# HIITMetagenomics/dsm-framework

Measured on AMD Instinct MI355X. Metric: enumerated substrings/sec (Emax=2.0), higher is better.
Workload: dtype u32

## Files before the change

### dsm-framework_amd/csrc/engine.hip

```cpp
#include <sched.h>

#include <algorithm>
#include <atomic>
#include <chrono>
#include <cmath>
#include <condition_variable>
#include <cstdlib>
#include <cstring>
#include <deque>
#include <map>
#include <functional>
#include <memory>
#include <mutex>
#include <sstream>
#include <thread>
#include <type_traits>

#include "common.h"
#include "scan.h"
#include "setorder.h"
#include "stream_parse.h"
#include "lfstep.h"
#include "entropy_tables.h"
#include "textemit.h"
// ... 194 lines not shown
#pragma unroll
        for (int g = 0; g < 8; ++g) {
            const u64 f = w[g] & (PACK_FMAX - 1);
            if (f) {
                const u32 lg = w[g] >> 13;
                l = l == 0xFF ? lg : (l == lg ? l : 5u);
                sumN += f;
                if (a.emax > 0) s += (double)(f + 1) * (double)__log2f((float)(f + 1));
            }
        }
    } else {
        for (u32 g = 0; g < a.d; ++g) {
            u64 f = (u64)x_freq<P>(x, g, v);
            if (f) {
                u32 lg = x_pl<P>(x, g, v) >> 4;
                l = l == 0xFF ? lg : (l == lg ? l : 5u);
                sumN += f;
                if (a.emax > 0) s += (double)(f + 1) * (double)__log2f((float)(f + 1));
            }
        }
    }
    if (l >= 1 && l <= 4) return false;
    if (a.emax > 0) {
        double e = (double)__log2f((float)sumN) - s / (double)sumN;
        if (e < a.emin - ENT_MARGIN || e > a.emax + ENT_MARGIN) return false;
    }
    return true;
}

constexpr u32 PW_CHUNK = 16;
constexpr u32 SREC_FIRST = 4u, SREC_LAST = 8u;
__device__ __forceinline__ uint2 child_path_word(const uint2 parent, u32 u, u32 plevel, u32 c) {
    const u32 r = plevel & (PW_CHUNK - 1);
    return r == 0 ? make_uint2(u, c) : make_uint2(parent.x, parent.y | (c << (2 * r)));
}

struct AdvanceOut {
    u32* slot;
    uint2* sa;
    uint2* pw;
    const uint2* parent_pw;
    const u32* width;
    u32 pw_after_slot;
    u32 plevel;
    u32 kshift;
    u32 cand_copy;
    u16* nT;
    u8* samechild;
    const u16* parent_nT;
    const u64* kplane;
    u64* kplane_w;
    u32* kcum;
    const u32* cnt4;
    u32* cnt_clear;
    u32 nbp;
    const u16* sinfo;
    u32 eval;
    u32 single;
    u32* const* rp;
    u32* rp0;
    const u64* const* splane;
    u32 rp_index;
    const u32* const* tpos;
    u32 nlocal, rank;
    u32 seg;
    u32 cap;
    u32* h_totals;
    u32 filter_on;
    FilterArgs fa;
    u64* candbits;
    u64* wsum;
    uint4* crec;
    u32 crec_cap;
};

struct PublishArgs {
    const u32* total;
    const u64* cand;
    const u8* cmax_base;
    u64 cmax_bpr;
    u32 cmax_world;
    u32* clear;
    u32* next;
    uint4* packet;
    u32 seq;
    uint4* bc_header;
    const u32* grand;
};
__global__ void publish_kernel(PublishArgs a) {
    __shared__ u32 wide;
    if (threadIdx.x == 0) wide = 0;
    __syncthreads();
    for (u32 r = threadIdx.x; r < a.cmax_world; r += blockDim.x) {
        const u64 m = *reinterpret_cast<const u64*>(a.cmax_base + (u64)r * a.cmax_bpr);
        if (m >= PACK_FMAX) atomicOr(&wide, m >= 65535 ? 3u : 2u);
    }
    const u32 tot = threadIdx.x == 0 ? *a.total : 0u;
    u64 cand = threadIdx.x == 0 && a.cand ? *a.cand : 0ull;
    if (threadIdx.x == 0 && a.grand) { const u64 c = (u64)(*a.grand - tot); cand = c | (c << 32); }
    __syncthreads();
    if (a.clear && threadIdx.x < 4) a.clear[threadIdx.x] = 0;
    if (threadIdx.x == 0) {
        if (a.next) { a.next[0] = tot; a.next[1] = wide; }
        const uint4 pk = make_uint4(a.seq, tot | ((wide & 1u) << 31) | ((wide >> 1) << 30), (u32)cand, (u32)(cand >> 32));
        if (a.bc_header) *a.bc_header = make_uint4(BC_OK, pk.y, 0u, 0u);
        *a.packet = pk;
// ... 203 lines not shown
    if (!o.single) o.samechild[u] = (u8)same;
#pragma unroll
    for (int c = 0; c < 4; ++c) {
        if (((pres >> c) & 1u) && vj[c] < o.cap) {
            if (o.slot) o.slot[vj[c]] = 4u * u + (u32)c;
            if (pw) pw[vj[c]] = child_path_word(mypw, u, o.plevel, (u32)c);
            if (o.sa) o.sa[vj[c]] = make_uint2(u, (u32)c | ((pres & ((1u << c) - 1u)) ? 0u : SREC_FIRST) | ((pres >> (c + 1)) ? 0u : SREC_LAST));
            if (!o.single) o.nT[vj[c]] = (u16)nT4[c];
        }
    }
    if (o.single) {
#pragma unroll
        for (int c = 0; c < 4; ++c)
            if (((pres >> c) & 1u) && vj[c] < o.cap) o.rp0[vj[c]] = (u32)c * o.seg + w * 64u + (u32)__popcll(up[c] & lt);
        return;
    }
    for (u32 sl = 0; sl < o.nlocal && pres && (o.tpos || o.rp_index); ++sl) {
        u32* rp = o.rp[sl];
        if (o.tpos) {
            const u32 m = x_pl<P>(x, o.rank * o.nlocal + sl, u) & 15u;
            const u32 h = m ? o.tpos[sl][u] : 0u;
#pragma unroll
            for (int c = 0; c < 4; ++c)
                if (((pres >> c) & 1u) && vj[c] < o.cap) rp[vj[c]] = ((m >> c) & 1u) ? h + (u32)__popc(m & ((1u << c) - 1u)) : DEAD;
        } else {
            const u64* sp = o.splane[sl] + (size_t)w * 4;
#pragma unroll
            for (int c = 0; c < 4; ++c) {
                if (!((pres >> c) & 1u) || vj[c] >= o.cap) continue;
                const u64 mine = sp[c];
                rp[vj[c]] = ((mine >> lane) & 1) ? (u32)c * o.seg + w * 64u + (u32)__popcll(mine & lt) : DEAD;
            }
        }
    }
}

template <typename P>
__global__ __launch_bounds__(256) void advance_single_kernel(Xchg x, AdvanceOut o) {
    const int lane = threadIdx.x & 63;
    const u32 F = (u32)x.F;
    const u32 nw = (F + 63) >> 6;
    const u32 tile = (u32)__builtin_amdgcn_readfirstlane((int)(xcd_block() * 4 + (threadIdx.x >> 6)));
    if (tile >= o.nbp) return;
    const u64 lt = (1ull << lane) - 1;
    const u64* __restrict__ line = o.kplane + (size_t)tile * 32;
    uint2 mypw[4];
#pragma unroll
    for (int q = 0; q < 4; ++q) {
        const u32 u = (tile * 4 + (u32)q) * 64 + lane;
        mypw[q] = o.parent_pw[u < F ? u : 0u];
    }
    u64 copyw = 0;
    if (lane < 32) copyw = line[lane];
    u32 cum[4];
#pragma unroll
    for (int c = 0; c < 4; ++c) cum[c] = o.cnt4[(size_t)c * o.nbp + tile];
    u64 up[4][4];
#pragma unroll
    for (int q = 0; q < 4; ++q)
#pragma unroll
        for (int c = 0; c < 4; ++c) up[q][c] = tile * 4 + (u32)q < nw ? line[q * 8 + c] : 0ull;
    {
        const u32 q = (u32)lane >> 3, j = (u32)lane & 7u, w = tile * 4 + q;
        if (lane < 32 && w < nw) {
            if (j < 4) o.kplane_w[(size_t)w * 4 + j] = copyw;
            else if (o.cand_copy && j == 4) o.candbits[w] = copyw;
            else if (o.cand_copy && j == 5) o.wsum[w] = copyw;
        }
    }
    const u32 r = o.plevel & (PW_CHUNK - 1);
    u32 kc = 0;
    u32 cbase = 0;
    u64 cbq[4] = {0, 0, 0, 0};
    u32 ncq[4] = {0, 0, 0, 0};
    u64 fq[4] = {0, 0, 0, 0};
    if (o.crec) {
        cbase = o.cnt4[(size_t)4 * o.nbp + tile] - o.cnt4[(size_t)4 * o.nbp];
#pragma unroll
        for (int q = 0; q < 4; ++q) {
            if (tile * 4 + (u32)q < nw) { cbq[q] = line[q * 8 + 4]; ncq[q] = (u32)line[q * 8 + 5]; }
            const u32 u = (tile * 4 + (u32)q) * 64 + lane;
            if ((cbq[q] >> lane) & 1ull) fq[q] = (u64)x_freq<P>(x, 0, u);
        }
    }
#pragma unroll
    for (int q = 0; q < 4; ++q) {
        const u32 w = tile * 4 + (u32)q, u = w * 64 + lane;
        const uint2 ppw = mypw[q];
        if (o.crec && cbq[q]) {
            const u32 k = cbase + bits_below_lane(cbq[q]);
            if (((cbq[q] >> lane) & 1ull) && k < o.crec_cap) o.crec[k] = make_uint4(u, 0u, (u32)fq[q], (u32)(fq[q] >> 32));
        }
        cbase += ncq[q];
#pragma unroll
        for (int c = 0; c < 4; ++c) {
            const u64 m = up[q][c];
            if (lane == q * 4 + c) kc = cum[c];
            const u32 below = bits_below_lane(m);
            const u32 vj = cum[c] + below;
            if (((m >> lane) & 1ull) && vj < o.cap) {
                o.rp0[vj] = (u32)c * o.seg + w * 64u + below;
                o.pw[vj] = r == 0 ? make_uint2(u, (u32)c) : make_uint2(ppw.x, ppw.y | ((u32)c << (2 * r)));
            }
            cum[c] += (u32)__popcll(m);
        }
    }
    if (lane < 16 && tile * 4 + ((u32)lane >> 2) < nw) o.kcum[(size_t)tile * 16 + lane] = kc;
}

__global__ __launch_bounds__(256) void lite_count_kernel(const u64* __restrict__ kplane, u32 nw, u32* __restrict__ cnt4, u32 nbp, u32 kshift, u32 cand_row = 0) {
    const u32 tile = blockIdx.x * 64 + (threadIdx.x >> 2), c = threadIdx.x & 3;
    if (tile >= nbp) return;
    u32 s = 0, nc = 0;
    if (cand_row && tile * 4 + c < nw) nc = (u32)kplane[((size_t)(tile * 4 + c) << 3) + 5];
#pragma unroll
    for (u32 q = 0; q < 4; ++q) {
        const u32 w = tile * 4 + q;
        if (w < nw) s += (u32)__popcll(kplane[((size_t)w << kshift) + c]);
    }
    cnt4[(size_t)c * nbp + tile] = s;
    if (cand_row) {
        nc += __shfl_xor(nc, 1, 64);
        nc += __shfl_xor(nc, 2, 64);
        if (c == 0) cnt4[(size_t)4 * nbp + tile] = nc;
    }
}
__global__ __launch_bounds__(256) void lite_slot_kernel(const u64* __restrict__ kplane, u32 F, const u32* __restrict__ cnt4, u32 nbp, u32 single_tile,
                                                        u32* __restrict__ slot, u32 cap) {
    const int lane = threadIdx.x & 63;
    const u32 nw = (F + 63) >> 6;
    const u32 tile = xcd_block();
    const u32 wi = threadIdx.x >> 6, w = tile * 4 + wi;
    if (w >= nw) return;
    const u32 u = w * 64 + lane;
    u32 base = 0;
#pragma unroll
    for (int c = 0; c < 4; ++c) {
        u32 before = 0, all = 0;
#pragma unroll
        for (u32 q = 0; q < 4; ++q) {
            const u32 wq = tile * 4 + q;
            const u32 t = wq < nw ? (u32)__popcll(kplane[(size_t)wq * 4 + c]) : 0u;
            before += q < wi ? t : 0u;
            all += t;
        }
        const u64 up = kplane[(size_t)w * 4 + c];
        const u32 first = (single_tile ? base : cnt4[(size_t)c * nbp + tile]) + before;
        base += all;
        const u32 vj = first + (u32)__popcll(up & ((1ull << lane) - 1));
        if (u < F && ((up >> lane) & 1) && vj < cap) slot[vj] = 4u * u + (u32)c;
    }
}

template <typename P>
__global__ __launch_bounds__(256) void order_kernel(u32 F, Xchg x, const u16* __restrict__ nT, const u64* __restrict__ order, Kids kids,
                                                    u64* __restrict__ order_next) {
    __shared__ u32 qn;
    __shared__ u32 qu[256];
    __shared__ u64 qm[256], qo[256];
    if (threadIdx.x == 0) qn = 0;
    __syncthreads();
    const u32 u = blockIdx.x * blockDim.x + threadIdx.x;
    if (u < F) {
        const u32 cnt = nT[u];
        const u64 ord = order[u];
        u64 mbyid = 0;
        u32 um = 0;
        if (x_is_nm8(x)) {
            u32 w[8];
            x_words8(x, u, w);
#pragma unroll
            for (int g = 0; g < 8; ++g) { const u32 m = (w[g] >> 9) & 15u; mbyid |= (u64)m << (4 * g); um |= m; }
        } else {
            for (u32 k = 0; k < cnt; ++k) {
                const u32 r = (u32)((ord >> (4 * k)) & 15);
                const u32 m = x_pl<P>(x, r, u) & 15u;
                mbyid |= (u64)m << (4 * r);
                um |= m;
// ... 1185 lines not shown
    tpos[i] = fc[r] + __popc(full & 15u & (low - 1));
}

#define EARENA_GET(var, T, n)                                                                       \
    do {                                                                                            \
        (var) = ea->template get<T>(n);                                                             \
        if (!(var)) return fail(DSM_E_CAPACITY, "device arena exhausted: use a longer prefix or a larger arena_bytes"); \
    } while (0)

template <typename P>
class Engine {
  public:
    std::vector<const dsm_index*> idx;
    std::vector<const dsm_trie*> tries;
    bool trie_mode = false;
    dsm_params prm;
    bool stream_mode = false;
    int nlocal = 0, world = 1, rank = 0;
    u32 d = 1;
    hipStream_t st = 0;
    int device = 0;

    u32 Fcap = 0;
    bool multi = false;
    bool owner_mode = false;
    bool is_owner = true;
    int owner = 0;
    u8* bc_buf = nullptr;
    u32* lite_slot[2] = {nullptr, nullptr};
    uint2* sa[2] = {nullptr, nullptr};
    u32 pub_seq = 0;
    u32 Seg = 0;
    u32 Rcap = 0;
    u32 FcapW = 0, SegW = 0, RcapW = 0;
    u32 seg_of(bool compact) const { return compact ? Seg : SegW; }
    u32* d_pub_tot = nullptr; u64* d_pub_cmax = nullptr;
    std::vector<P*> rec[2];
    std::vector<u32*> rp[2];
    std::vector<u32*> tpos;
    std::vector<u64*> splane;
    u32** d_rp_tab[2] = {nullptr, nullptr};
    u32** d_tpos_tab = nullptr;
    u64** d_splane_tab = nullptr;
    bool spec_mode = false;
    u32* d_dyn = nullptr;
    bool node_major(bool w9) const { return w9 && nlocal > 1 && nlocal <= 8 && !trie_mode; }
    u32 dense_min = 1u << 18;
    bool self_mode = false;
    std::vector<u64*> splane2;
    u8* xsend = nullptr;
    u8* xrecv[2] = {nullptr, nullptr};
    u64 bpr_cap = 0;
    u32 *cnt4 = nullptr, *scan_tmp = nullptr;
    u32* cntraw = nullptr;
    LfGeometry lfgeo{256, 16};
    u16* sinfo = nullptr;
    u16* nT[2] = {nullptr, nullptr};
    u8* samechild = nullptr;
    u64* order[2] = {nullptr, nullptr};
    u16* order16[2] = {nullptr, nullptr};
    u64 *cand_wsum = nullptr, *cand_wscan = nullptr, *scan_tmp64 = nullptr;
    u64* d_counters = nullptr;
    u32* d_totals = nullptr;
    u64* d_totals64 = nullptr;
    u32* h_totals = nullptr;
    u32* h_bounds = nullptr;
    u64* h_childmax = nullptr;
    std::vector<void*> owned;
    size_t owned_bytes = 0;
    Arena arena;
    Arena carena;
    Arena earena;
    Arena* ea = nullptr;
    hipEvent_t ev0 = nullptr, ev1 = nullptr;
    std::vector<hipEvent_t> evpool;
    dsm_stats stats;
    u32 splits = 0;
    Emitter emitter;
    dsm_text_sink text_sink_ = nullptr;

    ~Engine() {
        for (void* p : owned) (void)hipFree(p);
        if (h_totals) (void)hipHostFree(h_totals);
        if (h_bounds) (void)hipHostFree(h_bounds);
        if (h_childmax) (void)hipHostFree(h_childmax);
        if (ev0) (void)hipEventDestroy(ev0);
        if (ev1) (void)hipEventDestroy(ev1);
        {
            std::lock_guard<std::mutex> lk(g_expand_chain.mu);
            for (auto& kv : g_expand_chain.dev)
                if (kv.second.owner == this) kv.second = ExpandChain::Link();
        }
        for (hipEvent_t e : evpool) (void)hipEventDestroy(e);
        if (copy_stream) (void)hipStreamDestroy(copy_stream);
        if (fill_done) (void)hipEventDestroy(fill_done);
        for (auto e : chunk_filled) if (e) (void)hipEventDestroy(e);
        if (bounds_landed) (void)hipEventDestroy(bounds_landed);
    }

    template <class T> int dalloc(T*& p, size_t n) {
        void* q = nullptr;
        hipError_t e = hipMalloc(&q, (n ? n : 1) * sizeof(T));
        if (e != hipSuccess) return fail(DSM_E_NOMEM, std::string("hipMalloc: ") + hipGetErrorString(e));
        owned.push_back(q);
        owned_bytes += ((n ? n : 1) * sizeof(T) + 4095) & ~(size_t)4095;
        p = (T*)q;
        return 0;
    }

    int init(dsm_index* const* ix, int n, const dsm_params& p, bool stream) {
        device = ix[0]->device;
        u64 nsum = 0, nmax = 0;
        for (int k = 0; k < n; ++k) {
            if (ix[k]->device != device) return fail(DSM_E_INVAL, "all local indexes must live on one device");
            idx.push_back(ix[k]);
            nsum += ix[k]->meta.n;
            nmax = ix[k]->meta.n > nmax ? ix[k]->meta.n : nmax;
        }
        return init_common(n, p, stream, nsum, nmax);
    }
    int init_tries(dsm_trie* const* tr, int n, const dsm_params& p) {
        device = tr[0]->device;
        trie_mode = true;
        u64 nsum = 0, nmax = 0;
        for (int k = 0; k < n; ++k) {
            if (tr[k]->device != device) return fail(DSM_E_INVAL, "all tries must live on one device");
            tries.push_back(tr[k]);
            nsum += tr[k]->nodes + 16;
            nmax = tr[k]->nodes + 16 > nmax ? tr[k]->nodes + 16 : nmax;
        }
        return init_common(n, p, false, nsum, nmax);
    }
    int init_common(int n, const dsm_params& p, bool stream, u64 nsum, u64 nmax) {
        memset(&stats, 0, sizeof stats);
        prm = p;
        stream_mode = stream;
        nlocal = n;
        world = p.world_size > 1 ? (int)p.world_size : 1;
        rank = world > 1 ? (int)p.rank : 0;
        multi = world > 1 || (p.allgather && getenv("DSM_FORCE_EXCHANGE"));
        if (world > 1 && !p.allgather) return fail(DSM_E_INVAL, "world_size > 1 needs an allgather callback");
        owner_mode = multi && p.owner_mode != 0;
        if (owner_mode) {
            if (!p.gather || !p.bcast) return fail(DSM_E_INVAL, "owner_mode needs the gather and bcast callbacks");
            if ((int)p.owner_rank >= world) return fail(DSM_E_INVAL, "owner_rank >= world_size");
            if (stream || trie_mode) return fail(DSM_E_INVAL, "owner_mode is for mining indexes");
            owner = (int)p.owner_rank;
            is_owner = rank == owner;
        }
        if (rank >= world) return fail(DSM_E_INVAL, "rank >= world_size");
        if (n > MAX_LOCAL) return fail(DSM_E_INVAL, "at most 273 local samples per process");
        d = (u32)(world * nlocal);
        if (d > 273) return fail(DSM_E_INVAL, "too many samples (MAX_READERS 273, metaserver.cpp:19)");
        st = (hipStream_t)p.stream;
        DSM_HIP(hipSetDevice(device));
        size_t free_b = 0, total_b = 0;
        DSM_HIP(hipMemGetInfo(&free_b, &total_b));
        if (const char* e = getenv("DSM_DENSE_MIN")) dense_min = (u32)atol(e);
        spec_mode = d == 1 && !trie_mode && !multi;
        if (spec_mode) { if (int rc = dalloc(d_dyn, (size_t)4)) return rc; }
        self_mode = d > 1 && !trie_mode;
        if (owner_mode && !self_mode) return fail(DSM_E_INVAL, "owner_mode needs handles derived in the LF-step kernel (several samples)");
        const u64 fbound = (world > 1 ? (u64)d * nmax : nsum) + 16;
        u64 budget = p.arena_bytes ? p.arena_bytes : (u64)(free_b * 0.7);
        if (!p.arena_bytes) {
            u64 want = (256ull << 20) + 32ull * nsum * (u64)world;
            if (want < budget) budget = want;
        }
        if (budget > free_b) budget = (u64)(free_b * 0.9);
        const bool small_rec = sizeof(P) == 8 && !trie_mode;
        const u64 rec_b = small_rec ? 32 : REC_FIELDS * sizeof(P) + 1;
        u64 perF = (u64)nlocal * (2 * rec_b * 4 + 2 * 4 + 4 + 1)
                   + (u64)nlocal * (sizeof(P) + 1)
                   + 2ull * d * (sizeof(P) + 1)
                   + 2 * (2 + 1 + 8) + 1 + 16 + 64 + (d > 13 ? 4ull * d : 0) + (d > 1 ? 8 : 0);
        u64 fc = budget * (nlocal > 1 && !p.arena_bytes ? 2 : 1) / 3 / perF;
        if (fc > (1u << 28) - TILE) fc = (1u << 28) - TILE;
        if (fc < 512) return fail(DSM_E_NOMEM, "not enough device memory for the frontier buffers");
        if (fc > fbound) fc = fbound < 1024 ? 1024 : fbound;
        Fcap = (u32)fc;
        bpr_cap = (((u64)nlocal * Fcap * (sizeof(P) + 1) + 15) & ~15ull) + 16;
        if (p.exchange_send && p.exchange_recv && multi) {
            if (p.exchange_bytes < 1024) return fail(DSM_E_INVAL, "exchange buffers too small");
            u64 cap_slots = (p.exchange_bytes - 32) / ((u64)nlocal * (sizeof(P) + 1));
            if (cap_slots < Fcap) Fcap = (u32)cap_slots;
            bpr_cap = p.exchange_bytes;
            xsend = (u8*)p.exchange_send;
            xrecv[0] = (u8*)p.exchange_recv;
            xrecv[1] = (u8*)p.exchange_recv + (size_t)world * bpr_cap;
        } else {
            if (int rc = dalloc(xrecv[0], (size_t)world * bpr_cap)) return rc;
            if (int rc = dalloc(xrecv[1], (size_t)world * bpr_cap)) return rc;
            if (multi) { if (int rc = dalloc(xsend, (size_t)bpr_cap)) return rc; }
        }
        if (multi) {
            u64 mine = Fcap, agreed = 0;
            if (int rc = agree_min(mine, &agreed)) return rc;
            Fcap = (u32)agreed;
        }
        if (int rc = alloc_levels(small_rec)) return rc;
        const size_t used = owned_bytes;
        u64 arena_b = budget > used ? budget - used : 0;
        const u64 floor_b = p.arena_bytes ? (1u << 20) : (64u << 20);
        if (arena_b < floor_b) arena_b = floor_b;
        if (multi) {
            u64 agreed = 0;
            if (int rc = agree_min(arena_b, &agreed)) return rc;
            arena_b = agreed;
        }
        if (int rc = dalloc(arena.base, arena_b)) return rc;
        arena.cap = arena_b;
// ... 17 lines not shown
        DSM_HIP(hipEventCreateWithFlags(&ev1, hipEventDisableSystemFence));
        return 0;
    }

    int alloc_levels(bool small_rec) {
        Seg = (Fcap + TILE - 1) / TILE * TILE;
        Rcap = 4 * Seg;
        SegW = Seg; FcapW = Fcap;
        if (small_rec) {
            SegW = (u32)((u64)Seg * 32 / (REC_FIELDS * sizeof(P) + 1)) / TILE * TILE;
            if (SegW < TILE) SegW = TILE;
            FcapW = SegW < Fcap ? SegW : Fcap;
        }
        RcapW = 4 * SegW;
        const size_t rec_n = std::max(rec_elems<P>(RcapW), small_rec ? (size_t)Rcap * 32 / sizeof(P) : (size_t)0);
        const size_t ntile = Seg / TILE, nwave = ntile * 4;
        const u64 slots = (u64)Fcap * 4;
        for (int s = 0; s < nlocal; ++s) {
            P *a = nullptr, *b = nullptr;
            u32 *r0, *r1, *tp = nullptr;
            u64* pln = nullptr;
            if (!trie_mode) {
                if (int rc = dalloc(a, rec_n)) return rc;
                if (int rc = dalloc(b, rec_n)) return rc;
                if (int rc = dalloc(pln, nwave * (d == 1 ? 8 : 4))) return rc;
            } else {
                if (int rc = dalloc(tp, (size_t)Fcap)) return rc;
            }
            if (int rc = dalloc(r0, (size_t)Fcap)) return rc;
            if (int rc = dalloc(r1, (size_t)Fcap)) return rc;
            u64* pln2 = nullptr;
            if (self_mode) { if (int rc = dalloc(pln2, nwave * 4)) return rc; }
            splane2.push_back(pln2);
            rec[0].push_back(a); rec[1].push_back(b); rp[0].push_back(r0); rp[1].push_back(r1); tpos.push_back(tp); splane.push_back(pln);
        }
        for (int k = 0; k < 2; ++k) {
            if (int rc = dalloc(d_rp_tab[k], (size_t)nlocal)) return rc;
            DSM_HIP(hipMemcpy(d_rp_tab[k], rp[k].data(), (size_t)nlocal * sizeof(u32*), hipMemcpyHostToDevice));
        }
        if (int rc = dalloc(d_tpos_tab, (size_t)nlocal)) return rc;
        DSM_HIP(hipMemcpy(d_tpos_tab, tpos.data(), (size_t)nlocal * sizeof(u32*), hipMemcpyHostToDevice));
        if (int rc = dalloc(d_splane_tab, (size_t)nlocal)) return rc;
        DSM_HIP(hipMemcpy(d_splane_tab, splane.data(), (size_t)nlocal * sizeof(u64*), hipMemcpyHostToDevice));
        if (int rc = dalloc(cnt4, 5 * ntile + 8)) return rc;
        if (stream_mode)
            for (int k = 0; k < 2; ++k) if (int rc = dalloc(sa[k], (size_t)Fcap + 64)) return rc;
        if (owner_mode) {
            if (int rc = dalloc(bc_buf, 16 + 32 * nwave + 64)) return rc;
            for (int k = 0; k < 2; ++k) if (int rc = dalloc(lite_slot[k], (size_t)Fcap + 64)) return rc;
        }
        if (d == 1 && !trie_mode) {
            if (int rc = dalloc(cntraw, 5 * ntile + 8)) return rc;
            DSM_HIP(hipMemset(cntraw, 0, (5 * ntile + 8) * sizeof(u32)));
        }
        if (int rc = lf_step_geometry(sizeof(P) == 8, device, &lfgeo)) return rc;
        if (d > 1 || trie_mode) { if (int rc = dalloc(sinfo, (size_t)slots)) return rc; }
        if (int rc = dalloc(scan_tmp, scan_tmp_elems(5 * ntile) + 8)) return rc;
        for (int k = 0; k < 2; ++k) {
            if (int rc = dalloc(nT[k], Fcap)) return rc;
            if (int rc = dalloc(order[k], Fcap)) return rc;
        }
        if (d > 13)
            for (int k = 0; k < 2; ++k)
                if (int rc = dalloc(order16[k], (size_t)Fcap * d)) return rc;
        if (int rc = dalloc(samechild, Fcap)) return rc;
        if (int rc = dalloc(cand_wsum, nwave + 8)) return rc;
        if (int rc = dalloc(cand_wscan, nwave + 8)) return rc;
        if (int rc = dalloc(scan_tmp64, scan_tmp_elems(nwave) + 8)) return rc;
        if (int rc = dalloc(d_counters, (size_t)COUNTER_SHARDS * 8 + KEEP_FREQS / 64)) return rc;
        {
            std::vector<u32> kt(KEEP_FREQS / 32, ~0u);
            if (d == 1 && !trie_mode && prm.emax > 0) {
                const double* terms = term_table();
                const double* logn = logn_table();
                for (u32 f = 0; f < KEEP_FREQS; ++f) {
                    const u64 sumN = 1ull + f;
                    const double sl = f < TERM_TAB ? terms[f] : (double)((u64)f + 1) * log((double)((u64)f + 1)) / LN2;
                    const double e = (sumN < LOGN_TAB ? logn[sumN] : log((double)sumN) / LN2) - sl / (double)sumN;
                    if (e < prm.emin || e > prm.emax) kt[f >> 5] &= ~(1u << (f & 31));
                }
            }
            DSM_HIP(hipMemcpy(d_counters + (size_t)COUNTER_SHARDS * 8, kt.data(), kt.size() * sizeof(u32), hipMemcpyHostToDevice));
        }
        if (int rc = dalloc(d_totals, 8)) return rc;
        if (int rc = dalloc(d_totals64, 4)) return rc;
        if (int rc = dalloc(d_pub_tot, 8)) return rc;
        if (int rc = dalloc(d_pub_cmax, (size_t)(world > 0 ? world : 1))) return rc;
        DSM_HIP(hipHostMalloc((void**)&h_totals, 320 * sizeof(u32)));
        DSM_HIP(hipHostMalloc((void**)&h_bounds, 2 * (EmitSet::MAX_CHUNKS + 1) * sizeof(u32)));
        DSM_HIP(hipHostMalloc((void**)&h_childmax, (size_t)(world > 0 ? world : 1) * sizeof(u64)));
        return 0;
    }

    int agree_min(u64 mine, u64* out) {
        u8* send = xsend;
        DSM_HIP(hipMemcpyAsync(send, &mine, sizeof(u64), hipMemcpyHostToDevice, st));
        if (prm.allgather(prm.allgather_ctx, send, xrecv[0], sizeof(u64), (void*)st)) return fail(DSM_E_SINK, "allgather callback failed");
        std::vector<u64> all((size_t)world);
        DSM_HIP(hipMemcpyAsync(all.data(), xrecv[0], (size_t)world * sizeof(u64), hipMemcpyDeviceToHost, st));
        DSM_HIP(hipStreamSynchronize(st));
        u64 m = all[0];
        for (u64 v : all) m = v < m ? v : m;
        *out = m;
        return 0;
    }

// ... 41 lines not shown
            if (hipMemcpyAsync(e->bc_buf, hdr, 16, hipMemcpyHostToDevice, e->st) == hipSuccess) (void)hipStreamSynchronize(e->st);
            (void)e->prm.bcast(e->prm.owner_ctx, e->owner, e->bc_buf, bytes, (void*)e->st);
        }
    };

    u32 col_bytes(bool w16, bool w9) const { return w9 ? 2u : (w16 ? 3u : (u32)sizeof(P) + 1); }
    u64 level_bytes(u32 F, bool w16, bool w9) const { return (((u64)nlocal * F * col_bytes(w16, w9) + 15) & ~15ull) + 16; }
    static size_t bcast_bytes(u32 F) { return 16 + (size_t)((F + 63) >> 6) * 32; }
    u32 level_cap(bool w16) const { return w16 ? Fcap : FcapW; }
    int check_width(u32 Fn, bool w16) {
        if (Fn > level_cap(w16)) return fail(DSM_E_CAPACITY, "frontier wider than the device buffers: use a longer prefix or a larger arena_bytes");
        return 0;
    }
    u32 decode_level(u32 word, bool* w16, bool* w9) const {
        *w16 = !(word >> 31) && !trie_mode;
        *w9 = *w16 && !((word >> 30) & 1u);
        return word & 0x3FFFFFFFu;
    }
    int upload_order(int k, const u16* ro, size_t n) {
        if (d <= 13) {
            u64 ord = 0;
            for (size_t i = 0; i < n; ++i) ord |= (u64)ro[i] << (4 * i);
            DSM_HIP(hipMemcpyAsync(order[k], &ord, sizeof(u64), hipMemcpyHostToDevice, st));
        } else {
            DSM_HIP(hipMemcpyAsync(order16[k], ro, n * sizeof(u16), hipMemcpyHostToDevice, st));
        }
        return 0;
    }

    struct Walk {
        std::string prefix;
        RunOpts o;
        std::vector<LevelHost> L;
        u32 order_mode = 0;
        bool emitting = false;
        bool emit_failed = false;
        bool trace = false;
        size_t nev = 0;
        u32 F = 1, depth = 0;
        bool w16 = false, w9 = false;
        BcastGuard owed;
        explicit Walk(Engine* e) : owed(e) {}
        int cur() const { return (int)(depth & 1); }
    };
    struct Sweep {
        Xchg x;
        size_t mark = 0;
        u32* slot = nullptr;
        bool filtered = false;
        u32 crec_cap = 0;
        u32 Fn = 0;
        bool w16 = false, w9 = false;
        bool spec_hit = false;
    };

    int run(const char* prefix_c, dsm_tuple_sink tsink, dsm_byte_sink bsink, void* ctx, const RunOpts& o = RunOpts()) {
        Walk w(this);
        w.prefix = prefix_c ? prefix_c : "";
        w.o = o;
        for (char ch : w.prefix)
            if (ch != 'A' && ch != 'C' && ch != 'G' && ch != 'T')
                return fail(DSM_E_INVAL, "prefix must be over A,C,G,T");
        DSM_HIP(hipSetDevice(device));
        for (int s_ = 0; s_ < nlocal && !trie_mode; ++s_)
            if (!idx[s_]->dev.blk) return fail(DSM_E_INVAL, "an index of this miner is offloaded: dsm_index_reload first");
        arena.off = 0;
        earena.off = 0;
        carena.off = 0;
        w.emitting = o.emit;
        w.L.reserve(512);
        DSM_HIP(hipMemsetAsync(d_counters, 0, (size_t)COUNTER_SHARDS * 8 * sizeof(u64), st));
        if (cntraw) DSM_HIP(hipMemsetAsync(cntraw, 0, (4 * (size_t)(Seg / TILE) + 8) * sizeof(u32), st));
        DSM_HIP(hipEventRecord(ev0, st));
        if (int rc = root_level(w)) return rc;
        w.order_mode = (d < 2 || prm.pmax == 1) ? 0u : (d <= 13 ? 1u : 2u);
        stats.pair_order_exact = 1;
        w.trace = getenv("DSM_TRACE_LEVELS") != nullptr;
        DSM_HIP(hipMemsetAsync(multi ? xsend : xrecv[0], 0, XHDR, st));
        if (int rc = launch_lf(w, 0, 1, w.w16, w.w9, w.L[0].slot)) return rc;
        while (true) {
            if (int rc = exchange(w)) return rc;
            if (owner_mode && !is_owner) {
                bool more = false;
                if (int rc = client_level(w, &more)) return rc;
                if (!more) break;
                continue;
            }
            if (owner_mode) { if (int rc = owner_precheck(w)) return rc; }
            Sweep s;
            LevelHost child;
            if (int rc = advance(w, s)) return rc;
            if (int rc = publish(w, s)) return rc;
            if (int rc = commit(w, s, child)) return rc;
            if (int rc = capture_level(w, s.Fn, child.slot, child.pw)) return rc;
            if (s.filtered) {
                int erc = emit_store(w.L[w.depth], w.F, w.depth, s.x, w.cur(), w.order_mode, s.crec_cap);
                if (erc == DSM_E_CAPACITY && multi) { w.emit_failed = true; w.emitting = false; }
                else if (erc) return erc;
            }
            DSM_HIP(hipGetLastError());
            if (pend.submit && (w.F >= 200000u || w.depth >= 24)) { if (int rc = flush_pending()) return rc; }
            count_level(w);
            if (!s.Fn) break;
            w.L.push_back(child);
            step(w, s.Fn, s.w16, s.w9);
            if (w.L.size() > 60000) return fail(DSM_E_CAPACITY, "trie deeper than 60000 levels");
        }
        timeline("levels done", w.prefix.c_str());
        if (int rc = flush_pending()) return rc;
        if (int rc = finish_prefix(w, tsink, bsink, ctx)) return rc;
        if (w.o.last && pend.submit) {
            DSM_HIP(hipEventSynchronize(bounds_landed));
            if (int rc = flush_pending()) return rc;
        }
        return read_back(w);
    }

    int root_level(Walk& w) {
        const char* bases = "ACGT";
        for (int s = 0; s < nlocal && trie_mode; ++s) {
            const u32 zero = 0;
            DSM_HIP(hipMemcpyAsync(rp[0][s], &zero, sizeof(u32), hipMemcpyHostToDevice, st));
            stats.reported += tries[s]->nodes;
        }
        for (int s = 0; s < nlocal && !trie_mode; ++s) {
// ... 231 lines not shown
            ARENA_GET(me.clen, u8, F);
            hipLaunchKernelGGL((keep_kernel<P>), grid_for(F), dim3(256), 0, st, F, x, sa[cur], me.srec, me.clen);
        }
        if (!stream_mode && w.emitting && depth >= 1 && depth >= w.o.emit_lo && depth <= w.o.emit_hi) {
            int erc = emit_alloc(me, F);
            if (erc == DSM_E_CAPACITY && multi) { w.emit_failed = true; w.emitting = false; }
            else if (erc) return erc;
            else s.filtered = true;
        }
        s.mark = arena.off;
        const bool keep_slot = self_mode, keep_pw = !stream_mode;
        const size_t wcap = (size_t)F * 4 < Fcap ? (size_t)F * 4 : Fcap;
        u8* window = arena.get<u8>(wcap * ((keep_slot ? 4 : 0) + (keep_pw ? 8 : 0)) + 512);
        if (!window) return fail(DSM_E_CAPACITY, "device arena exhausted: use a longer prefix or a larger arena_bytes");
        s.slot = keep_slot ? reinterpret_cast<u32*>(window) : nullptr;
        const u32 nbp = (F + TILE - 1) / TILE;
        AdvanceOut ao;
        memset(&ao, 0, sizeof ao);
        ao.slot = s.slot; ao.nT = nT[nxt]; ao.samechild = samechild;
        if (stream_mode) ao.sa = sa[nxt];
        if (keep_pw) {
            ao.pw = reinterpret_cast<uint2*>(window);
            ao.pw_after_slot = keep_slot ? 1u : 0u;
            ao.parent_pw = me.pw;
            ao.plevel = depth;
        }
        ao.parent_nT = nT[cur]; ao.nlocal = (u32)nlocal; ao.rank = (u32)rank;
        ao.cap = (u32)wcap;
        ao.seg = seg_of(w.w16 && !trie_mode);
        ao.h_totals = d_pub_tot;
        ao.rp = d_rp_tab[nxt];
        ao.rp0 = rp[nxt][0];
        ao.tpos = trie_mode ? d_tpos_tab : nullptr;
        ao.splane = d_splane_tab;
        ao.rp_index = self_mode ? 0u : 1u;
        ao.kcum = me.kcum; ao.cnt4 = cnt4; ao.nbp = nbp; ao.kshift = 2;
        ao.width = d_totals;
        const bool merged = d > 1 || trie_mode;
        if (merged && nbp == 1) {
            ao.eval = 1; ao.kplane_w = me.kplane;
        } else if (merged) {
            hipLaunchKernelGGL((advance_reduce_kernel<P>), dim3(nbp), dim3(256), 0, st, x, sinfo, me.kplane, cnt4, nbp);
            ao.kplane = me.kplane; ao.sinfo = sinfo;
        } else {
            ao.kplane = splane[0]; ao.kplane_w = me.kplane; ao.single = 1;
            ao.kshift = 3;
        }
        const bool lean = !merged && nbp > 1 && keep_pw && !keep_slot && !stream_mode;
        if (lean && s.filtered && carena.cap) {
            const size_t room = (carena.cap - carena.off) / sizeof(uint4);
            s.crec_cap = (u32)(room < (size_t)F ? room : (size_t)F);
        }
        const bool fold = s.crec_cap > 0;
        if (nbp > 1) {
            if (!merged) hipLaunchKernelGGL(lite_count_kernel, dim3((nbp + 63) / 64), dim3(256), 0, st, splane[0], (F + 63) >> 6, cntraw, nbp, 3u, fold ? 1u : 0u);
            exclusive_scan<u32, u32>(merged ? cnt4 : cntraw, cnt4, (size_t)(fold ? 5 : 4) * nbp, scan_tmp, d_totals, st);
        }
        const bool fused_filter = s.filtered && nbp > 1;
        if (fused_filter) {
            ao.fa = filter_args(F, depth, w.order_mode); ao.candbits = me.cand_bits; ao.wsum = cand_wsum;
            if (ao.single) ao.cand_copy = 1;
            else ao.filter_on = 1;
        }
        if (fold) { ao.crec = reinterpret_cast<uint4*>(carena.base + carena.off); ao.crec_cap = s.crec_cap; }
        if (nbp == 1) hipLaunchKernelGGL((advance_down_kernel<P>), dim3(1), dim3(256), 0, st, x, ao);
        else if (lean) hipLaunchKernelGGL((advance_single_kernel<P>), dim3((nbp + 3) / 4), dim3(256), 0, st, x, ao);
        else hipLaunchKernelGGL((advance_wave_kernel<P>), dim3(nbp), dim3(256), 0, st, x, ao);
        if (s.filtered) {
            if (int erc = emit_filter(me, F, depth, x, cur, w.order_mode, !fused_filter, fold)) return erc;
        }
        return 0;
    }

    int publish(Walk& w, Sweep& s) {
        const u32 F = w.F, nbp = (F + TILE - 1) / TILE;
        const int nxt = w.cur() ^ 1;
        PublishArgs pa;
        memset(&pa, 0, sizeof pa);
        pa.total = nbp == 1 ? d_pub_tot : d_totals;
        pa.cmax_base = s.x.base; pa.cmax_bpr = s.x.bpr; pa.cmax_world = (u32)world;
        if (s.filtered) pa.cand = d_totals64;
        if (s.crec_cap) {
            pa.total = cnt4 + (size_t)4 * nbp;
            pa.grand = d_totals;
            pa.cand = nullptr;
        }
        pa.clear = reinterpret_cast<u32*>(multi ? xsend : xrecv[nxt]);
        pa.packet = reinterpret_cast<uint4*>(h_totals + 304); pa.seq = ++pub_seq;
        pa.next = spec_mode ? d_dyn : nullptr;
        pa.bc_header = owner_mode ? reinterpret_cast<uint4*>(bc_buf) : nullptr;
        hipLaunchKernelGGL(publish_kernel, dim3(1), dim3(64), 0, st, pa);
        if (owner_mode) {
            const size_t bc_bytes = bcast_bytes(F);
            DSM_HIP(hipMemcpyAsync(bc_buf + 16, w.L[w.depth].kplane, bc_bytes - 16, hipMemcpyDeviceToDevice, st));
            w.owed.disarm();
            if (prm.bcast(prm.owner_ctx, owner, bc_buf, bc_bytes, (void*)st)) return fail(DSM_E_SINK, "bcast callback failed");
            stats.exchange_bytes_sent += bc_bytes * (u64)(world - 1);
        }
        if (spec_mode) { if (int rc = launch_lf(w, w.depth + 1, 0, w.w16, w.w9, s.slot, (u64)F * 4)) return rc; }
        u32 pk[4];
        if (int rc = wait_packet(pk)) return rc;
        s.Fn = decode_level(pk[1], &s.w16, &s.w9);
        s.spec_hit = spec_mode && s.Fn > 0 && s.Fn <= level_cap(s.w16) && s.w16 == w.w16 && s.w9 == w.w9;
        if (spec_mode && !s.spec_hit) --stats.expand_launches;
        h_totals[300] = pk[2]; h_totals[301] = pk[3];
        if (int rc = check_width(s.Fn, s.w16)) return rc;
        if (owner_mode) {
            if (!s.Fn) w.owed.arm(16);
            else w.owed.arm_next((size_t)level_bytes(s.Fn, s.w16, s.w9), xrecv[nxt], bcast_bytes(s.Fn));
        }
        return 0;
    }
    int wait_packet(u32 pk[4]) {
        volatile u32* fl = h_totals + 304;
        u32 spins = 0;
        while (*fl != pub_seq) {
            if ((++spins & 0xFFFFu) == 0 && hipStreamQuery(st) != hipErrorNotReady) {
                DSM_HIP(hipStreamSynchronize(st));
                if (*fl != pub_seq) return fail(DSM_E_HIP, "publish kernel did not report");
                break;
            }
            __builtin_ia32_pause();
        }
        std::atomic_thread_fence(std::memory_order_acquire);
        for (int q = 0; q < 4; ++q) pk[q] = fl[q];
        return 0;
    }

    int commit(Walk& w, const Sweep& s, LevelHost& child) {
        const u32 F = w.F, Fn = s.Fn;
        const int cur = w.cur(), nxt = cur ^ 1;
        arena.off = s.mark;
        child.n = Fn;
        if (!Fn) return 0;
        if (self_mode) child.slot = arena.get<u32>(Fn);
        if (!stream_mode) child.pw = arena.get<uint2>(Fn);
        if (int rc = alloc_kids(child)) return rc;
        if (s.spec_hit) {
            stats.expand_slots += Fn;
            stats.expand_column_bytes += (u64)Fn * col_bytes(s.w16, s.w9);
        } else {
            if (int rc = launch_lf(w, w.depth + 1, Fn, s.w16, s.w9, child.slot)) return rc;
        }
        const Kids kids = w.L[w.depth].kids();
// ... 744 lines not shown
```

Measured before the change: 3.966 billion.

## Fuse lean-path tile counting, scan, and publish into one level-offsets kernel

On the lean single-process path, the separate lite_count kernel, multi-pass exclusive_scan and publish kernel are replaced by one level_offsets_kernel. Each block scans a range of tiles locally and writes per-block totals. The last-arriving block, detected with an atomic counter, scans those totals into per-block offsets and writes the publish packet directly. advance_single_kernel then adds the block offset, found through a magic-number division, to its tile-local prefix. This cuts kernel launches and global passes per level, at the cost of a serialized last-block scan and added atomic and fence synchronisation.

```diff
diff --git a/dsm-framework_amd/csrc/engine.hip b/dsm-framework_amd/csrc/engine.hip
--- a/dsm-framework_amd/csrc/engine.hip
+++ b/dsm-framework_amd/csrc/engine.hip
@@ -270,6 +270,8 @@
     u64* kplane_w;
     u32* kcum;
     const u32* cnt4;
+    const u32* boff;
+    u32 bmagic;
     u32* cnt_clear;
     u32 nbp;
     const u16* sinfo;
@@ -579,9 +581,15 @@
     }
     u64 copyw = 0;
     if (lane < 32) copyw = line[lane];
-    u32 cum[4];
+    const u32 blk = o.bmagic ? __umulhi(tile, o.bmagic) : tile;
+    u32 cum[4], cumb[5];
 #pragma unroll
     for (int c = 0; c < 4; ++c) cum[c] = o.cnt4[(size_t)c * o.nbp + tile];
+#pragma unroll
+    for (int c = 0; c < 5; ++c) cumb[c] = o.boff[(size_t)blk * 8 + c];
+    u32 cbase = o.cnt4[(o.crec ? 4u : 0u) * o.nbp + tile] + cumb[4];
+#pragma unroll
+    for (int c = 0; c < 4; ++c) cum[c] += cumb[c];
     u64 up[4][4];
 #pragma unroll
     for (int q = 0; q < 4; ++q)
@@ -597,12 +605,10 @@
     }
     const u32 r = o.plevel & (PW_CHUNK - 1);
     u32 kc = 0;
-    u32 cbase = 0;
     u64 cbq[4] = {0, 0, 0, 0};
     u32 ncq[4] = {0, 0, 0, 0};
     u64 fq[4] = {0, 0, 0, 0};
     if (o.crec) {
-        cbase = o.cnt4[(size_t)4 * o.nbp + tile] - o.cnt4[(size_t)4 * o.nbp];
 #pragma unroll
         for (int q = 0; q < 4; ++q) {
             if (tile * 4 + (u32)q < nw) { cbq[q] = line[q * 8 + 4]; ncq[q] = (u32)line[q * 8 + 5]; }
@@ -651,6 +657,121 @@
         nc += __shfl_xor(nc, 2, 64);
         if (c == 0) cnt4[(size_t)4 * nbp + tile] = nc;
     }
+}
+constexpr u32 LEVEL_GMAX = 4096;
+constexpr u32 LVL_ITEMS = 8;
+constexpr u32 LVL_GTARGET = 128;
+constexpr u32 LVL_COUNT = 0, LVL_GRAND = 16, LVL_WIDTH = 17, LVL_WORDS = 32;
+struct LevelOffArgs {
+    const u64* kplane;
+    u32 nw, nbp;
+    u32 B, G;
+    u32 fold;
+    u32* cnt4;
+    u32* bsum;
+    u32* boff;
+    u32* sync;
+    u32 publish;
+    PublishArgs pa;
+};
+__global__ __launch_bounds__(256) void level_offsets_kernel(LevelOffArgs a) {
+    __shared__ u32 wtot[4][5];
+    __shared__ u32 last;
+    const u32 lane = threadIdx.x & 63, w = threadIdx.x >> 6;
+    const u32 t0 = blockIdx.x * a.B, t1 = t0 + a.B < a.nbp ? t0 + a.B : a.nbp;
+    u32 run[5] = {0, 0, 0, 0, 0};
+    for (u32 tb = t0; tb < t1; tb += 256) {
+        const u32 tile = tb + threadIdx.x;
+        const bool in = tile < t1;
+        ulonglong2 p[4][2];
+        u64 ncw[4] = {0, 0, 0, 0};
+#pragma unroll
+        for (u32 q = 0; q < 4; ++q) {
+            const u32 wq = in && tile * 4 + q < a.nw ? tile * 4 + q : 0u;
+            const ulonglong2* line = reinterpret_cast<const ulonglong2*>(a.kplane + ((size_t)wq << 3));
+            p[q][0] = line[0];
+            p[q][1] = line[1];
+            if (a.fold) ncw[q] = a.kplane[((size_t)wq << 3) + 5];
+        }
+        u32 s[5] = {0, 0, 0, 0, 0};
+#pragma unroll
+        for (u32 q = 0; q < 4; ++q) {
+            if (!(in && tile * 4 + q < a.nw)) continue;
+            s[0] += (u32)__popcll(p[q][0].x); s[1] += (u32)__popcll(p[q][0].y);
+            s[2] += (u32)__popcll(p[q][1].x); s[3] += (u32)__popcll(p[q][1].y);
+            s[4] += (u32)ncw[q];
+        }
+        u32 inc[5];
+#pragma unroll
+        for (int c = 0; c < 5; ++c) inc[c] = wave_inclusive_scan(s[c]);
+        if (lane == 63) {
+#pragma unroll
+            for (int c = 0; c < 5; ++c) wtot[w][c] = inc[c];
+        }
+        __syncthreads();
+#pragma unroll
+        for (int c = 0; c < 5; ++c) {
+            u32 before = 0, all = 0;
+#pragma unroll
+            for (u32 k = 0; k < 4; ++k) { const u32 t = wtot[k][c]; before += k < w ? t : 0u; all += t; }
+            if (in && (c < 4 || a.fold)) a.cnt4[(size_t)c * a.nbp + tile] = run[c] + before + inc[c] - s[c];
+            run[c] += all;
+        }
+        __syncthreads();
+    }
+    const u32 nrow = a.fold ? 5u : 4u;
+    u32 width = 0, ncand = 0;
+    if (a.G == 1) {
+        if (threadIdx.x == 0) {
+            a.boff[0] = 0; a.boff[1] = run[0]; a.boff[2] = run[0] + run[1]; a.boff[3] = run[0] + run[1] + run[2];
+            a.boff[4] = 0;
+        }
+        width = run[0] + run[1] + run[2] + run[3];
+        ncand = run[4];
+    } else {
+        if (threadIdx.x == 0) {
+            for (u32 c = 0; c < nrow; ++c) a.bsum[(size_t)c * a.G + blockIdx.x] = c == 4 ? run[4] : DSM_PICK(run, c);
+            __builtin_amdgcn_fence(__ATOMIC_RELEASE, "agent");
+            last = __hip_atomic_fetch_add(a.sync + LVL_COUNT, 1u, __ATOMIC_RELAXED, __HIP_MEMORY_SCOPE_AGENT) == a.G - 1 ? 1u : 0u;
+        }
+        __syncthreads();
+        if (!last) return;
+        __builtin_amdgcn_fence(__ATOMIC_ACQUIRE, "agent");
+        for (u32 row0 = 0; row0 < nrow; row0 += 4) {
+            const u32 n = (row0 ? 1u : 4u) * a.G, at = row0 * a.G;
+            u32 carry = 0;
+            for (u32 i0 = 0; i0 < n; i0 += 256 * LVL_ITEMS) {
+                const u32 base = i0 + threadIdx.x * LVL_ITEMS;
+                u32 v[LVL_ITEMS], sum = 0;
+#pragma unroll
+                for (u32 k = 0; k < LVL_ITEMS; ++k) {
+                    v[k] = base + k < n ? __hip_atomic_load(a.bsum + at + base + k, __ATOMIC_RELAXED, __HIP_MEMORY_SCOPE_AGENT) : 0u;
+                    sum += v[k];
+                }
+                u32 tot;
+                u32 ex = carry + block_exclusive_scan<u32>(sum, &tot);
+                u32 c = base / a.G, b = base - c * a.G;
+#pragma unroll
+                for (u32 k = 0; k < LVL_ITEMS; ++k) {
+                    if (base + k < n) a.boff[(size_t)b * 8 + row0 + c] = ex;
+                    ex += v[k];
+                    if (++b == a.G) { b = 0; ++c; }
+                }
+                carry += tot;
+            }
+            if (row0) ncand = carry; else width = carry;
+        }
+        if (threadIdx.x == 0) __hip_atomic_store(a.sync + LVL_COUNT, 0u, __ATOMIC_RELAXED, __HIP_MEMORY_SCOPE_AGENT);
+    }
+    if (threadIdx.x != 0) return;
+    a.sync[LVL_GRAND] = width + ncand;
+    a.sync[LVL_WIDTH] = width;
+    if (!a.publish) return;
+    const u64 m = *reinterpret_cast<const u64*>(a.pa.cmax_base);
+    const u32 wide = m >= PACK_FMAX ? (m >= 65535 ? 3u : 2u) : 0u;
+    if (a.pa.clear) { a.pa.clear[0] = 0; a.pa.clear[1] = 0; a.pa.clear[2] = 0; a.pa.clear[3] = 0; }
+    if (a.pa.next) { a.pa.next[0] = width; a.pa.next[1] = wide; }
+    *a.pa.packet = make_uint4(a.pa.seq, width | ((wide & 1u) << 31) | ((wide >> 1) << 30), ncand, ncand);
 }
 __global__ __launch_bounds__(256) void lite_slot_kernel(const u64* __restrict__ kplane, u32 F, const u32* __restrict__ cnt4, u32 nbp, u32 single_tile,
                                                         u32* __restrict__ slot, u32 cap) {
@@ -1942,6 +2063,8 @@
     u8* xrecv[2] = {nullptr, nullptr};
     u64 bpr_cap = 0;
     u32 *cnt4 = nullptr, *scan_tmp = nullptr;
+    u32 *lvl_bsum = nullptr, *lvl_boff = nullptr, *lvl_sync = nullptr;
+    u32 level_block_tiles = 0;
     u32* cntraw = nullptr;
     LfGeometry lfgeo{256, 16};
     u16* sinfo = nullptr;
@@ -2047,6 +2170,7 @@
         size_t free_b = 0, total_b = 0;
         DSM_HIP(hipMemGetInfo(&free_b, &total_b));
         if (const char* e = getenv("DSM_DENSE_MIN")) dense_min = (u32)atol(e);
+        if (const char* e = getenv("DSM_LEVEL_BLOCK_TILES")) level_block_tiles = (u32)atol(e);
         spec_mode = d == 1 && !trie_mode && !multi;
         if (spec_mode) { if (int rc = dalloc(d_dyn, (size_t)4)) return rc; }
         self_mode = d > 1 && !trie_mode;
@@ -2170,6 +2294,10 @@
         if (d == 1 && !trie_mode) {
             if (int rc = dalloc(cntraw, 5 * ntile + 8)) return rc;
             DSM_HIP(hipMemset(cntraw, 0, (5 * ntile + 8) * sizeof(u32)));
+            if (int rc = dalloc(lvl_bsum, (size_t)5 * LEVEL_GMAX)) return rc;
+            if (int rc = dalloc(lvl_boff, (size_t)8 * LEVEL_GMAX)) return rc;
+            if (int rc = dalloc(lvl_sync, (size_t)LVL_WORDS)) return rc;
+            DSM_HIP(hipMemset(lvl_sync, 0, LVL_WORDS * sizeof(u32)));
         }
         if (int rc = lf_step_geometry(sizeof(P) == 8, device, &lfgeo)) return rc;
         if (d > 1 || trie_mode) { if (int rc = dalloc(sinfo, (size_t)slots)) return rc; }
@@ -2317,6 +2445,8 @@
         u32 Fn = 0;
         bool w16 = false, w9 = false;
         bool spec_hit = false;
+        bool lean = false;
+        bool published = false;
     };
 
     int run(const char* prefix_c, dsm_tuple_sink tsink, dsm_byte_sink bsink, void* ctx, const RunOpts& o = RunOpts()) {
@@ -2336,6 +2466,7 @@
         w.L.reserve(512);
         DSM_HIP(hipMemsetAsync(d_counters, 0, (size_t)COUNTER_SHARDS * 8 * sizeof(u64), st));
         if (cntraw) DSM_HIP(hipMemsetAsync(cntraw, 0, (4 * (size_t)(Seg / TILE) + 8) * sizeof(u32), st));
+        if (lvl_sync) DSM_HIP(hipMemsetAsync(lvl_sync, 0, LVL_WORDS * sizeof(u32), st));
         DSM_HIP(hipEventRecord(ev0, st));
         if (int rc = root_level(w)) return rc;
         w.order_mode = (d < 2 || prm.pmax == 1) ? 0u : (d <= 13 ? 1u : 2u);
@@ -2673,7 +2804,24 @@
             s.crec_cap = (u32)(room < (size_t)F ? room : (size_t)F);
         }
         const bool fold = s.crec_cap > 0;
-        if (nbp > 1) {
+        s.lean = lean;
+        if (lean) {
+            u32 B = level_block_tiles ? level_block_tiles : 256u;
+            if (!level_block_tiles) while ((nbp + B - 1) / B > LVL_GTARGET) B <<= 1;
+            if ((nbp + B - 1) / B > LEVEL_GMAX) B = (nbp + LEVEL_GMAX - 1) / LEVEL_GMAX;
+            if ((B & (B - 1)) && (u64)nbp * B >= (1ull << 32)) { u32 b2 = 1; while (b2 < B) b2 <<= 1; B = b2; }
+            LevelOffArgs la;
+            memset(&la, 0, sizeof la);
+            la.kplane = splane[0]; la.nw = (F + 63) >> 6; la.nbp = nbp; la.B = B; la.G = (nbp + B - 1) / B; la.fold = fold ? 1u : 0u;
+            la.cnt4 = cnt4; la.bsum = lvl_bsum; la.boff = lvl_boff; la.sync = lvl_sync;
+            ao.boff = lvl_boff;
+            ao.bmagic = B == 1 ? 0u : (u32)((1ull << 32) / B) + ((B & (B - 1)) ? 1u : 0u);
+            if (!multi && !owner_mode && (!s.filtered || fold)) {
+                la.publish = 1; la.pa = publish_args(w, s);
+                s.published = true;
+            }
+            hipLaunchKernelGGL(level_offsets_kernel, dim3(la.G), dim3(256), 0, st, la);
+        } else if (nbp > 1) {
             if (!merged) hipLaunchKernelGGL(lite_count_kernel, dim3((nbp + 63) / 64), dim3(256), 0, st, splane[0], (F + 63) >> 6, cntraw, nbp, 3u, fold ? 1u : 0u);
             exclusive_scan<u32, u32>(merged ? cnt4 : cntraw, cnt4, (size_t)(fold ? 5 : 4) * nbp, scan_tmp, d_totals, st);
         }
@@ -2693,7 +2841,7 @@
         return 0;
     }
 
-    int publish(Walk& w, Sweep& s) {
+    PublishArgs publish_args(const Walk& w, const Sweep& s) {
         const u32 F = w.F, nbp = (F + TILE - 1) / TILE;
         const int nxt = w.cur() ^ 1;
         PublishArgs pa;
@@ -2701,16 +2849,23 @@
         pa.total = nbp == 1 ? d_pub_tot : d_totals;
         pa.cmax_base = s.x.base; pa.cmax_bpr = s.x.bpr; pa.cmax_world = (u32)world;
         if (s.filtered) pa.cand = d_totals64;
-        if (s.crec_cap) {
-            pa.total = cnt4 + (size_t)4 * nbp;
-            pa.grand = d_totals;
-            pa.cand = nullptr;
+        if (s.lean) {
+            pa.total = lvl_sync + LVL_WIDTH;
+            if (s.crec_cap) {
+                pa.grand = lvl_sync + LVL_GRAND;
+                pa.cand = nullptr;
+            }
         }
         pa.clear = reinterpret_cast<u32*>(multi ? xsend : xrecv[nxt]);
         pa.packet = reinterpret_cast<uint4*>(h_totals + 304); pa.seq = ++pub_seq;
         pa.next = spec_mode ? d_dyn : nullptr;
         pa.bc_header = owner_mode ? reinterpret_cast<uint4*>(bc_buf) : nullptr;
-        hipLaunchKernelGGL(publish_kernel, dim3(1), dim3(64), 0, st, pa);
+        return pa;
+    }
+    int publish(Walk& w, Sweep& s) {
+        const u32 F = w.F;
+        const int nxt = w.cur() ^ 1;
+        if (!s.published) hipLaunchKernelGGL(publish_kernel, dim3(1), dim3(64), 0, st, publish_args(w, s));
         if (owner_mode) {
             const size_t bc_bytes = bcast_bytes(F);
             DSM_HIP(hipMemcpyAsync(bc_buf + 16, w.L[w.depth].kplane, bc_bytes - 16, hipMemcpyDeviceToDevice, st));
```

Result: slower. 3.658 billion (-7.8%).
